# abcouwer-jpl/zsc

Hardware: AMD Instinct MI355X
Metric: deflate level-6 uncompressed MB/s in, Canterbury-like x4096 per GPU (higher is better)
Workload: dtype u8

## Files before the change

### __graft_entry__.py

```python
from __future__ import annotations

import os
import subprocess
import sys

ROOT = os.path.dirname(os.path.abspath(__file__))
if ROOT not in sys.path:
    sys.path.insert(0, ROOT)


def build() -> None:
    subprocess.run(["make", "-s", "-C", os.path.join(ROOT, "zsc_amd", "csrc")], check=True)
    subprocess.run(["make", "-s", "-C", os.path.join(ROOT, "oracle"), "oracle", "ref"], check=True)
    subprocess.run(["make", "-s", "-C", os.path.join(ROOT, "tests", "emu")], check=True)
    subprocess.run(["make", "-s", "-C", os.path.join(ROOT, "tests", "emu_sections")], check=True)
    subprocess.run(["make", "-s", "-C", os.path.join(ROOT, "tests", "emu_chunks")], check=True)
    subprocess.run(["make", "-s", "-C", os.path.join(ROOT, "tests", "emu_resync")], check=True)
    subprocess.run(["make", "-s", "-C", os.path.join(ROOT, "tests", "emu_index")], check=True)
    subprocess.run(["make", "-s", "-C", os.path.join(ROOT, "tests", "emu_size")], check=True)
    subprocess.run(["make", "-s", "-C", os.path.join(ROOT, "tests", "emu_check")], check=True)
    subprocess.run(["make", "-s", "-C", os.path.join(ROOT, "tests", "emu_dindex")], check=True)
    subprocess.run(["make", "-s", "-C", os.path.join(ROOT, "tests", "emu_verify")], check=True)
    subprocess.run(["make", "-s", "-C", os.path.join(ROOT, "tests", "emu_pack")], check=True)
    subprocess.run(["make", "-s", "-C", os.path.join(ROOT, "tests", "emu_pipe")], check=True)
    subprocess.run(["make", "-s", "-C", os.path.join(ROOT, "tests", "emu_sort")], check=True)
    subprocess.run(["make", "-s", "-C", os.path.join(ROOT, "tests", "emu_lazy")], check=True)
    subprocess.run(["make", "-s", "-C", os.path.join(ROOT, "tests", "c_caller")], check=True)
    import zsc_amd


def smoke() -> None:
    import zsc_amd
    from zsc_amd import corpus
    from oracle.oracle_py import Oracle

    print("device:", zsc_amd.device_info())
    oracle = Oracle()
    bufs = [corpus.make_buffer(kind, size, 7 + i) for i, (kind, size) in enumerate(
        [("text", 70000), ("bitmap", 40000), ("table", 20000), ("random", 5000), ("zero", 3000),
         ("token", 257), ("text", 0)])]
    rc, outs, stats = zsc_amd.compress_batch(bufs, level=6)
    assert rc == 0, rc
    for i, (src, got, st) in enumerate(zip(bufs, outs, stats)):
        orc, want, _ = oracle.compress(src, 6)
        assert st == orc == 0, (i, st, orc)
        assert got == want, f"buffer {i}: GPU stream differs from the oracle ({len(got)} vs {len(want)} bytes)"
    rc, one = zsc_amd.compress(bufs[0], level=9)
    assert rc == 0 and one == oracle.compress(bufs[0], 9)[1]
    rc, back, used, istat = zsc_amd.uncompress_batch(outs, [len(b) for b in bufs])
    assert rc == 0 and all(s == 0 for s in istat), (rc, istat)
    assert back == bufs and used == [len(o) for o in outs]
    print("smoke ok:", [len(o) for o in outs])


if __name__ == "__main__":
    build()
    if len(sys.argv) > 1 and sys.argv[1] == "smoke":
        smoke()
```

### zsc_amd/csrc/huff_plan.h

```cpp
#ifndef ZSC_HUFF_PLAN_H
#define ZSC_HUFF_PLAN_H

#include "wave.h"
#include "zsc_dev.h"

#define HP_LCODES 286
#define HP_DCODES 30
#define HP_BLCODES 19
#define HP_HEAP (2 * HP_LCODES + 1)

typedef struct {
    uint32_t freq[HP_HEAP];
    uint16_t parent[HP_HEAP];
    uint16_t len[HP_HEAP];
    uint16_t code[HP_HEAP];
    int max_code;
} HpTree;

typedef struct {
    uint32_t freq[2 * HP_DCODES + 1];
    uint16_t parent[2 * HP_DCODES + 1];
    uint16_t len[2 * HP_DCODES + 2];
    uint16_t code[2 * HP_DCODES + 1];
    int max_code;
} HpTreeD;

typedef struct {
    uint32_t freq[2 * HP_BLCODES + 1];
    uint16_t parent[2 * HP_BLCODES + 1];
    uint16_t len[2 * HP_BLCODES + 1];
    uint16_t code[2 * HP_BLCODES + 1];
    int max_code;
} HpTreeB;

typedef struct {
    HpTree lt;
    HpTreeD dt;
    HpTreeB bt;
    uint16_t heap[HP_HEAP];
    uint8_t depth[HP_HEAP];
    uint16_t per_len[16];
    uint32_t opt_bits, static_bits;
    int heap_n, heap_top;
    uint8_t hdr[ZD_HDR_BYTES];
    uint32_t hdr_acc, hdr_fill, hdr_pos;
} HpLds;

typedef struct {
    uint32_t *freq;
    uint16_t *parent, *len, *code;
    int *max_code;
    int elems, max_len, extra_from, has_static, is_dist;
    int kind;
} HpView;

DEV int hp_extra(int kind, int sym)
{
    if (kind == 0) {
        if (sym < 265 || sym == 285)
            return 0;
        return (sym - 261) >> 2;
    }
    if (kind == 1)
        return sym < 4 ? 0 : (sym >> 1) - 1;
    return sym == 16 ? 2 : sym == 17 ? 3 : sym == 18 ? 7 : 0;
}

DEV uint32_t hp_static_llen(uint32_t c)
{
    return c < 144 ? 8u : c < 256 ? 9u : c < 280 ? 7u : 8u;
}

DEV uint32_t hp_len_code(uint32_t lc)
{
    if (lc < 8)
        return lc;
    if (lc == 255)
        return 28;
    uint32_t e = 29u - (uint32_t)__builtin_clz(lc);
    return 4u * e + 4u + ((lc >> e) & 3u);
}

DEV uint32_t hp_dist_code(uint32_t d)
{
    if (d < 4)
        return d;
    uint32_t e = 30u - (uint32_t)__builtin_clz(d);
    return 2u * e + 2u + ((d >> e) & 1u);
}

DEV uint32_t hp_len_base(uint32_t c)
{
    if (c < 8)
        return c;
    if (c == 28)
        return 0;
    uint32_t e = (c - 4) >> 2;
    return (4u + ((c - 4) & 3u)) << e;
}

DEV uint32_t hp_dist_base(uint32_t c)
{
    if (c < 4)
        return c;
    uint32_t e = (c >> 1) - 1;
    return (2u + (c & 1u)) << e;
}

DEV uint32_t hp_bitrev(uint32_t v, int bits)
{
    uint32_t r = 0;
    while (bits-- > 0) {
        r = (r << 1) | (v & 1u);
        v >>= 1;
    }
    return r;
}

DEV int hp_before(const HpView &t, const uint8_t *depth, int a, int b)
{
    return t.freq[a] < t.freq[b] || (t.freq[a] == t.freq[b] && depth[a] <= depth[b]);
}

DEV void hp_sift(HpLds *h, const HpView &t, int k)
{
    int v = h->heap[k];
    for (int j = k << 1; j <= h->heap_n; j <<= 1) {
        if (j < h->heap_n && hp_before(t, h->depth, h->heap[j + 1], h->heap[j]))
            j++;
        if (hp_before(t, h->depth, v, h->heap[j]))
            break;
        h->heap[k] = h->heap[j];
        k = j;
    }
    h->heap[k] = (uint16_t)v;
}

DEV void hp_build(HpLds *h, const HpView &t)
{
    int top = -1;
    h->heap_n = 0;
    h->heap_top = HP_HEAP;
    for (int n = 0; n < t.elems; n++) {
        if (t.freq[n]) {
            h->heap[++h->heap_n] = (uint16_t)(top = n);
            h->depth[n] = 0;
        } else {
            t.len[n] = 0;
        }
    }
    while (h->heap_n < 2) {
        int node = top < 2 ? ++top : 0;
        h->heap[++h->heap_n] = (uint16_t)node;
        t.freq[node] = 1;
        h->depth[node] = 0;
        h->opt_bits--;
        if (t.has_static)
            h->static_bits -= t.is_dist ? 5u : hp_static_llen((uint32_t)node);
    }
    *t.max_code = top;
    for (int n = h->heap_n / 2; n >= 1; n--)
        hp_sift(h, t, n);

    int node = t.elems;
    do {
        int a = h->heap[1];
        h->heap[1] = h->heap[h->heap_n--];
        hp_sift(h, t, 1);
        int b = h->heap[1];
        h->heap[--h->heap_top] = (uint16_t)a;
        h->heap[--h->heap_top] = (uint16_t)b;
        t.freq[node] = t.freq[a] + t.freq[b];
        h->depth[node] = (uint8_t)((h->depth[a] >= h->depth[b] ? h->depth[a] : h->depth[b]) + 1);
        t.parent[a] = t.parent[b] = (uint16_t)node;
        h->heap[1] = (uint16_t)node++;
        hp_sift(h, t, 1);
    } while (h->heap_n >= 2);
    h->heap[--h->heap_top] = h->heap[1];

    int over = 0;
    for (int b = 0; b < 16; b++)
        h->per_len[b] = 0;
    t.len[h->heap[h->heap_top]] = 0;
    int i;
    for (i = h->heap_top + 1; i < HP_HEAP; i++) {
        int n = h->heap[i];
        int bits = t.len[t.parent[n]] + 1;
        if (bits > t.max_len) {
            bits = t.max_len;
            over++;
        }
        t.len[n] = (uint16_t)bits;
        if (n > top)
            continue;
        h->per_len[bits]++;
        int xb = n >= t.extra_from ? hp_extra(t.kind, n) : 0;
        h->opt_bits += t.freq[n] * (uint32_t)(bits + xb);
        if (t.has_static)
            h->static_bits += t.freq[n] * ((t.is_dist ? 5u : hp_static_llen((uint32_t)n)) + (uint32_t)xb);
    }
    if (over > 0) {
        do {
            int bits = t.max_len - 1;
            while (h->per_len[bits] == 0)
                bits--;
            h->per_len[bits]--;
            h->per_len[bits + 1] += 2;
            h->per_len[t.max_len]--;
            over -= 2;
        } while (over > 0);
        for (int bits = t.max_len; bits != 0; bits--) {
            int n = h->per_len[bits];
            while (n != 0) {
                int m = h->heap[--i];
                if (m > top)
                    continue;
                if (t.len[m] != (uint16_t)bits) {
                    h->opt_bits += ((uint32_t)bits - t.len[m]) * t.freq[m];
                    t.len[m] = (uint16_t)bits;
                }
                n--;
            }
        }
    }
    uint16_t next[16];
    uint32_t code = 0;
    for (int b = 1; b <= 15; b++) {
        code = (code + h->per_len[b - 1]) << 1;
        next[b] = (uint16_t)code;
    }
    for (int n = 0; n <= top; n++) {
        int l = t.len[n];
        if (l)
            t.code[n] = (uint16_t)hp_bitrev(next[l]++, l);
    }
}

DEV void hp_scan(HpLds *h, uint16_t *len, int max_code)
{
    int prev = -1, next = len[0], count = 0, hi = 7, lo = 4;
    if (next == 0) {
        hi = 138;
        lo = 3;
    }
    len[max_code + 1] = 0xffff;
    for (int n = 0; n <= max_code; n++) {
        int cur = next;
        next = len[n + 1];
        if (++count < hi && cur == next)
            continue;
        if (count < lo)
            h->bt.freq[cur] += (uint32_t)count;
        else if (cur != 0) {
            if (cur != prev)
                h->bt.freq[cur]++;
            h->bt.freq[16]++;
        } else if (count <= 10)
            h->bt.freq[17]++;
        else
            h->bt.freq[18]++;
        count = 0;
        prev = cur;
        if (next == 0) {
            hi = 138;
            lo = 3;
        } else if (cur == next) {
            hi = 6;
            lo = 3;
        } else {
            hi = 7;
            lo = 4;
        }
    }
}

DEV void hp_put(HpLds *h, uint32_t value, int nbits)
{
    h->hdr_acc |= value << h->hdr_fill;
    h->hdr_fill += (uint32_t)nbits;
    while (h->hdr_fill >= 8) {
        h->hdr[h->hdr_pos++] = (uint8_t)h->hdr_acc;
        h->hdr_acc >>= 8;
        h->hdr_fill -= 8;
    }
}

DEV void hp_send_lengths(HpLds *h, const uint16_t *len, int max_code)
{
    int prev = -1, next = len[0], count = 0, hi = 7, lo = 4;
    if (next == 0) {
        hi = 138;
        lo = 3;
    }
    for (int n = 0; n <= max_code; n++) {
        int cur = next;
        next = len[n + 1];
        if (++count < hi && cur == next)
            continue;
        if (count < lo) {
            do
                hp_put(h, h->bt.code[cur], h->bt.len[cur]);
            while (--count != 0);
        } else if (cur != 0) {
            if (cur != prev) {
                hp_put(h, h->bt.code[cur], h->bt.len[cur]);
                count--;
            }
            hp_put(h, h->bt.code[16], h->bt.len[16]);
            hp_put(h, (uint32_t)(count - 3), 2);
        } else if (count <= 10) {
            hp_put(h, h->bt.code[17], h->bt.len[17]);
            hp_put(h, (uint32_t)(count - 3), 3);
        } else {
            hp_put(h, h->bt.code[18], h->bt.len[18]);
            hp_put(h, (uint32_t)(count - 11), 7);
        }
        count = 0;
        prev = cur;
        if (next == 0) {
            hi = 138;
            lo = 3;
        } else if (cur == next) {
            hi = 6;
            lo = 3;
        } else {
            hi = 7;
            lo = 4;
        }
    }
}

DEV void huff_plan_block(const uint32_t *syms, const ZdBlockRec *rec, uint32_t strategy,
                         ZdBlockPlan *plan, HpLds *h)
{
    const uint32_t count = rec->sym_count;
    for (int i = 0; i < HP_HEAP; i += WAVE) {
        FOR_LANES
        {
            if (i + LANE < HP_HEAP)
                h->lt.freq[i + LANE] = 0;
        }
    }
    FOR_LANES
    {
        if (LANE < 2 * HP_DCODES + 1)
            h->dt.freq[LANE] = 0;
        if (LANE < 2 * HP_BLCODES + 1)
            h->bt.freq[LANE] = 0;
    }
    for (uint32_t s = 0; s < count; s += WAVE) {
        FOR_LANES
        {
            uint32_t i = s + (uint32_t)LANE;
            if (i < count) {
                uint32_t v = syms[i];
                uint32_t dist = v >> 16, lc = v & 0xff;
                if (dist == 0) {
                    LDS_ADD_U32(&h->lt.freq[lc], 1u);
                } else {
                    LDS_ADD_U32(&h->lt.freq[257 + hp_len_code(lc)], 1u);
                    LDS_ADD_U32(&h->dt.freq[hp_dist_code(dist - 1)], 1u);
                }
            }
        }
    }
    WAVE_SYNC();
    int last_bl = 0;
    uint32_t type = ZD_BT_DYNAMIC;
    ON_LANE0
    {
        h->lt.freq[256] = 1;
        h->opt_bits = h->static_bits = 0;
        HpView vl = {h->lt.freq, h->lt.parent, h->lt.len, h->lt.code, &h->lt.max_code,
                     HP_LCODES, 15, 257, 1, 0, 0};
        HpView vd = {h->dt.freq, h->dt.parent, h->dt.len, h->dt.code, &h->dt.max_code,
                     HP_DCODES, 15, 0, 1, 1, 1};
        HpView vb = {h->bt.freq, h->bt.parent, h->bt.len, h->bt.code, &h->bt.max_code,
                     HP_BLCODES, 7, 0, 0, 0, 2};
        hp_build(h, vl);
        hp_build(h, vd);
        hp_scan(h, h->lt.len, h->lt.max_code);
        hp_scan(h, h->dt.len, h->dt.max_code);
        hp_build(h, vb);
        const uint8_t order[19] = {16, 17, 18, 0, 8, 7, 9, 6, 10, 5, 11, 4, 12, 3, 13, 2, 14, 1, 15};
        for (last_bl = HP_BLCODES - 1; last_bl >= 3; last_bl--)
            if (h->bt.len[order[last_bl]] != 0)
                break;
        h->opt_bits += 3u * ((uint32_t)last_bl + 1u) + 5u + 5u + 4u;

        uint32_t opt_bytes = (h->opt_bits + 3 + 7) >> 3;
        const uint32_t static_bytes = (h->static_bits + 3 + 7) >> 3;
        if (static_bytes <= opt_bytes)
            opt_bytes = static_bytes;
        if (rec->in_len + 4 <= opt_bytes && rec->stored_ok)
            type = ZD_BT_STORED;
        else if (strategy == 4 || static_bytes == opt_bytes)
            type = ZD_BT_STATIC;
        else
            type = ZD_BT_DYNAMIC;

        h->hdr_acc = h->hdr_fill = h->hdr_pos = 0;
        if (type == ZD_BT_DYNAMIC) {
            hp_put(h, (uint32_t)(h->lt.max_code + 1 - 257), 5);
            hp_put(h, (uint32_t)(h->dt.max_code + 1 - 1), 5);
            hp_put(h, (uint32_t)(last_bl + 1 - 4), 4);
            for (int r = 0; r <= last_bl; r++)
                hp_put(h, h->bt.len[order[r]], 3);
            hp_send_lengths(h, h->lt.len, h->lt.max_code);
            hp_send_lengths(h, h->dt.len, h->dt.max_code);
        }
        plan->type = type;
        plan->hdr_bits = h->hdr_pos * 8 + h->hdr_fill;
        if (h->hdr_fill)
            h->hdr[h->hdr_pos] = (uint8_t)h->hdr_acc;
        plan->body_bits = type == ZD_BT_DYNAMIC ? 3u + h->opt_bits
                          : type == ZD_BT_STATIC ? 3u + h->static_bits : 0u;
        plan->bit_off = 0;
    }
    WAVE_SYNC();
    for (int i = 0; i < HP_LCODES; i += WAVE) {
        FOR_LANES
        {
            int s = i + LANE;
            if (s < HP_LCODES) {
                int used = s <= h->lt.max_code && h->lt.len[s] != 0;
                plan->lcode[s] = used ? h->lt.code[s] : (uint16_t)0;
                plan->llen[s] = used ? (uint8_t)h->lt.len[s] : (uint8_t)0;
            }
        }
    }
    FOR_LANES
    {
        if (LANE < HP_DCODES) {
            int used = LANE <= h->dt.max_code && h->dt.len[LANE] != 0;
            plan->dcode[LANE] = used ? h->dt.code[LANE] : (uint16_t)0;
            plan->dlen[LANE] = used ? (uint8_t)h->dt.len[LANE] : (uint8_t)0;
        }
    }
    for (int i = 0; i < (int)ZD_HDR_BYTES; i += WAVE) {
        FOR_LANES
        {
            if (i + LANE < (int)ZD_HDR_BYTES)
                plan->hdr[i + LANE] = h->hdr[i + LANE];
        }
    }
}

#endif
```

Before: 7576.

## Parallelize Huffman plan construction across the wave with packed heap keys

Reworks per-block Huffman tree planning. Heap entries become packed freq/depth/node words, so comparisons are single integer compares and the parent arrays go away. Leaf collection, bit-cost sums and canonical code assignment now run across all lanes using ballot, popcount and wave reductions instead of serial loops on lane 0. The histogram loop issues several symbol loads per lane, and the header bit writer flushes 32-bit words straight into the plan. It also adds an emulator test target. The risk is packed-field overflow (frequency capped near 2^17, checked only by an emulator assert) and subtle tie-break changes that could break bit-exactness with the oracle.

```diff
diff --git a/__graft_entry__.py b/__graft_entry__.py
--- a/__graft_entry__.py
+++ b/__graft_entry__.py
@@ -25,6 +25,7 @@
     subprocess.run(["make", "-s", "-C", os.path.join(ROOT, "tests", "emu_pipe")], check=True)
     subprocess.run(["make", "-s", "-C", os.path.join(ROOT, "tests", "emu_sort")], check=True)
     subprocess.run(["make", "-s", "-C", os.path.join(ROOT, "tests", "emu_lazy")], check=True)
+    subprocess.run(["make", "-s", "-C", os.path.join(ROOT, "tests", "emu_huff")], check=True)
     subprocess.run(["make", "-s", "-C", os.path.join(ROOT, "tests", "c_caller")], check=True)
     import zsc_amd
 
diff --git a/zsc_amd/csrc/huff_plan.h b/zsc_amd/csrc/huff_plan.h
--- a/zsc_amd/csrc/huff_plan.h
+++ b/zsc_amd/csrc/huff_plan.h
@@ -3,56 +3,64 @@
 
 #include "wave.h"
 #include "zsc_dev.h"
+#ifdef ZSC_WAVE_EMU
+#include <assert.h>
+#define HP_ASSERT(x) assert(x)
+#else
+#define HP_ASSERT(x) ((void)0)
+#endif
+
+#ifndef HP_PATH
+#define HP_PATH(id) ((void)0)
+#endif
 
 #define HP_LCODES 286
 #define HP_DCODES 30
 #define HP_BLCODES 19
 #define HP_HEAP (2 * HP_LCODES + 1)
 
+#define HP_NODE_MASK 1023u
+#define HP_WORD(freq, depth, node) (((uint32_t)(freq) << 15) | ((uint32_t)(depth) << 10) | (uint32_t)(node))
+#define HP_KEY(w) ((w) >> 10)
+#define HP_FREQ(w) ((w) >> 15)
+#define HP_DEPTH(w) (((w) >> 10) & 31u)
+#define HP_NO_SYM 0xffffffffu
+#ifndef HP_HIST_LOADS
+#define HP_HIST_LOADS 4
+#endif
+
 typedef struct {
-    uint32_t freq[HP_HEAP];
-    uint16_t parent[HP_HEAP];
-    uint16_t len[HP_HEAP];
-    uint16_t code[HP_HEAP];
-    int max_code;
-} HpTree;
-
-typedef struct {
-    uint32_t freq[2 * HP_DCODES + 1];
-    uint16_t parent[2 * HP_DCODES + 1];
-    uint16_t len[2 * HP_DCODES + 2];
-    uint16_t code[2 * HP_DCODES + 1];
-    int max_code;
-} HpTreeD;
-
-typedef struct {
-    uint32_t freq[2 * HP_BLCODES + 1];
-    uint16_t parent[2 * HP_BLCODES + 1];
-    uint16_t len[2 * HP_BLCODES + 1];
-    uint16_t code[2 * HP_BLCODES + 1];
-    int max_code;
-} HpTreeB;
-
-typedef struct {
-    HpTree lt;
-    HpTreeD dt;
-    HpTreeB bt;
-    uint16_t heap[HP_HEAP];
-    uint8_t depth[HP_HEAP];
-    uint16_t per_len[16];
-    uint32_t opt_bits, static_bits;
-    int heap_n, heap_top;
-    uint8_t hdr[ZD_HDR_BYTES];
-    uint32_t hdr_acc, hdr_fill, hdr_pos;
+    uint32_t heap[HP_HEAP + 1];
+    uint32_t lfreq[HP_LCODES];
+    uint32_t dfreq[HP_DCODES];
+    uint32_t bfreq[HP_BLCODES];
+    uint32_t bsend[HP_BLCODES];
+    uint32_t per_len[16];
+    uint8_t llen[HP_HEAP + 3];
+    uint8_t dlen[2 * HP_DCODES + 4];
+    uint8_t blen[2 * HP_BLCODES + 2];
 } HpLds;
 
-typedef struct {
-    uint32_t *freq;
-    uint16_t *parent, *len, *code;
-    int *max_code;
-    int elems, max_len, extra_from, has_static, is_dist;
-    int kind;
-} HpView;
+template <int KIND> struct HpTree;
+template <> struct HpTree<0> {
+    enum { elems = HP_LCODES, max_len = 15, has_static = 1 };
+};
+template <> struct HpTree<1> {
+    enum { elems = HP_DCODES, max_len = 15, has_static = 1 };
+};
+template <> struct HpTree<2> {
+    enum { elems = HP_BLCODES, max_len = 7, has_static = 0 };
+};
+
+DEV uint32_t *hp_freq(HpLds *h, int kind)
+{
+    return kind == 0 ? h->lfreq : kind == 1 ? h->dfreq : h->bfreq;
+}
+
+DEV uint8_t *hp_len(HpLds *h, int kind)
+{
+    return kind == 0 ? h->llen : kind == 1 ? h->dlen : h->blen;
+}
 
 DEV int hp_extra(int kind, int sym)
 {
@@ -117,148 +125,246 @@
     return r;
 }
 
-DEV int hp_before(const HpView &t, const uint8_t *depth, int a, int b)
-{
-    return t.freq[a] < t.freq[b] || (t.freq[a] == t.freq[b] && depth[a] <= depth[b]);
-}
-
-DEV void hp_sift(HpLds *h, const HpView &t, int k)
-{
-    int v = h->heap[k];
-    for (int j = k << 1; j <= h->heap_n; j <<= 1) {
-        if (j < h->heap_n && hp_before(t, h->depth, h->heap[j + 1], h->heap[j]))
+DEV void hp_sift(uint32_t *heap, int n, int k, uint32_t v)
+{
+    for (int j = k << 1; j <= n; j <<= 1) {
+        uint32_t c = heap[j];
+        const uint32_t c1 = heap[j + 1];
+        if (j < n && HP_KEY(c1) <= HP_KEY(c)) {
+            c = c1;
             j++;
-        if (hp_before(t, h->depth, v, h->heap[j]))
+        }
+        if (HP_KEY(v) <= HP_KEY(c))
             break;
-        h->heap[k] = h->heap[j];
+        heap[k] = c;
         k = j;
     }
-    h->heap[k] = (uint16_t)v;
-}
-
-DEV void hp_build(HpLds *h, const HpView &t)
-{
-    int top = -1;
-    h->heap_n = 0;
-    h->heap_top = HP_HEAP;
-    for (int n = 0; n < t.elems; n++) {
-        if (t.freq[n]) {
-            h->heap[++h->heap_n] = (uint16_t)(top = n);
-            h->depth[n] = 0;
-        } else {
-            t.len[n] = 0;
-        }
-    }
-    while (h->heap_n < 2) {
-        int node = top < 2 ? ++top : 0;
-        h->heap[++h->heap_n] = (uint16_t)node;
-        t.freq[node] = 1;
-        h->depth[node] = 0;
-        h->opt_bits--;
-        if (t.has_static)
-            h->static_bits -= t.is_dist ? 5u : hp_static_llen((uint32_t)node);
-    }
-    *t.max_code = top;
-    for (int n = h->heap_n / 2; n >= 1; n--)
-        hp_sift(h, t, n);
-
-    int node = t.elems;
+    heap[k] = v;
+}
+
+template <int KIND>
+DEV void hp_heap_and_lengths(HpLds *h, int n, int top)
+{
+    typedef HpTree<KIND> T;
+    uint32_t *heap = h->heap;
+    uint8_t *len = hp_len(h, KIND);
+    for (int k = n / 2; k >= 1; k--)
+        hp_sift(heap, n, k, heap[k]);
+
+    int node = T::elems, ht = HP_HEAP;
     do {
-        int a = h->heap[1];
-        h->heap[1] = h->heap[h->heap_n--];
-        hp_sift(h, t, 1);
-        int b = h->heap[1];
-        h->heap[--h->heap_top] = (uint16_t)a;
-        h->heap[--h->heap_top] = (uint16_t)b;
-        t.freq[node] = t.freq[a] + t.freq[b];
-        h->depth[node] = (uint8_t)((h->depth[a] >= h->depth[b] ? h->depth[a] : h->depth[b]) + 1);
-        t.parent[a] = t.parent[b] = (uint16_t)node;
-        h->heap[1] = (uint16_t)node++;
-        hp_sift(h, t, 1);
-    } while (h->heap_n >= 2);
-    h->heap[--h->heap_top] = h->heap[1];
+        const uint32_t a = heap[1];
+        const uint32_t last = heap[n];
+        n--;
+        hp_sift(heap, n, 1, last);
+        const uint32_t b = heap[1];
+        heap[--ht] = ((uint32_t)node << 10) | (a & HP_NODE_MASK);
+        heap[--ht] = ((uint32_t)node << 10) | (b & HP_NODE_MASK);
+        const uint32_t da = HP_DEPTH(a), db = HP_DEPTH(b);
+        const uint32_t depth = (da >= db ? da : db) + 1u, freq = HP_FREQ(a) + HP_FREQ(b);
+        HP_ASSERT(depth < 32u && freq < (1u << 17));
+        hp_sift(heap, n, 1, HP_WORD(freq, depth, node));
+        node++;
+    } while (n >= 2);
+    const int root = (int)(heap[1] & HP_NODE_MASK);
 
     int over = 0;
-    for (int b = 0; b < 16; b++)
-        h->per_len[b] = 0;
-    t.len[h->heap[h->heap_top]] = 0;
-    int i;
-    for (i = h->heap_top + 1; i < HP_HEAP; i++) {
-        int n = h->heap[i];
-        int bits = t.len[t.parent[n]] + 1;
-        if (bits > t.max_len) {
-            bits = t.max_len;
+    len[root] = 0;
+    uint32_t w = heap[ht];
+    for (int i = ht; i < HP_HEAP; i++) {
+        const uint32_t wn = heap[i + 1];
+        int bits = len[w >> 10] + 1;
+        if (bits > (int)T::max_len) {
+            bits = T::max_len;
             over++;
         }
-        t.len[n] = (uint16_t)bits;
-        if (n > top)
-            continue;
-        h->per_len[bits]++;
-        int xb = n >= t.extra_from ? hp_extra(t.kind, n) : 0;
-        h->opt_bits += t.freq[n] * (uint32_t)(bits + xb);
-        if (t.has_static)
-            h->static_bits += t.freq[n] * ((t.is_dist ? 5u : hp_static_llen((uint32_t)n)) + (uint32_t)xb);
+        len[w & HP_NODE_MASK] = (uint8_t)bits;
+        w = wn;
     }
     if (over > 0) {
+        HP_PATH(1 + KIND);
+        uint32_t *per_len = h->per_len;
+        for (int b = 0; b < 16; b++)
+            per_len[b] = 0;
+        for (int i = ht; i < HP_HEAP; i++) {
+            const int m = (int)(heap[i] & HP_NODE_MASK);
+            if (m <= top)
+                per_len[len[m]]++;
+        }
         do {
-            int bits = t.max_len - 1;
-            while (h->per_len[bits] == 0)
+            int bits = T::max_len - 1;
+            while (per_len[bits] == 0)
                 bits--;
-            h->per_len[bits]--;
-            h->per_len[bits + 1] += 2;
-            h->per_len[t.max_len]--;
+            per_len[bits]--;
+            per_len[bits + 1] += 2;
+            per_len[T::max_len]--;
             over -= 2;
         } while (over > 0);
-        for (int bits = t.max_len; bits != 0; bits--) {
-            int n = h->per_len[bits];
-            while (n != 0) {
-                int m = h->heap[--i];
+        int i = HP_HEAP;
+        for (int bits = T::max_len; bits != 0; bits--) {
+            uint32_t k = per_len[bits];
+            while (k != 0) {
+                const int m = (int)(heap[--i] & HP_NODE_MASK);
                 if (m > top)
                     continue;
-                if (t.len[m] != (uint16_t)bits) {
-                    h->opt_bits += ((uint32_t)bits - t.len[m]) * t.freq[m];
-                    t.len[m] = (uint16_t)bits;
+                len[m] = (uint8_t)bits;
+                k--;
+            }
+        }
+    }
+}
+
+template <int KIND>
+DEV int hp_build(HpLds *h, ZdBlockPlan *plan, uint32_t &opt_bits, uint32_t &static_bits)
+{
+    typedef HpTree<KIND> T;
+    enum { NCH = (T::elems + WAVE - 1) / WAVE };
+    uint32_t *const freq = hp_freq(h, KIND);
+    uint8_t *const len = hp_len(h, KIND);
+    int top = -1, n = 0;
+    for (int c = 0; c < NCH; c++) {
+        LANEVAR(uint32_t, f);
+        FOR_LANES
+        {
+            const int s = c * WAVE + LANE;
+            LV(f) = s < (int)T::elems ? freq[s] : 0u;
+            if (s < (int)T::elems)
+                len[s] = 0;
+        }
+        const uint64_t m = BALLOT(f);
+        FOR_LANES
+        {
+            if (LV(f))
+                h->heap[n + 1 + POPC64(m & ((1ull << LANE) - 1ull))] = HP_WORD(LV(f), 0, c * WAVE + LANE);
+        }
+        if (m) {
+            n += POPC64(m);
+            top = c * WAVE + 63 - CLZ64(m);
+        }
+    }
+    while (n < 2) {
+        HP_PATH(0);
+        const int node = top < 2 ? ++top : 0;
+        n++;
+        ON_LANE0
+        {
+            h->heap[n] = HP_WORD(1, 0, node);
+            freq[node] = 1;
+        }
+        opt_bits--;
+        if (T::has_static)
+            static_bits -= KIND == 1 ? 5u : hp_static_llen((uint32_t)node);
+    }
+    WAVE_SYNC();
+    ON_LANE0
+    {
+        hp_heap_and_lengths<KIND>(h, n, top);
+    }
+    WAVE_SYNC();
+
+    LANEARR(uint32_t, ln, NCH);
+    LANEARR(uint32_t, cd, NCH);
+    LANEVAR(uint64_t, bits);
+    FOR_LANES
+    {
+        LV(bits) = 0;
+    }
+    UNROLL_FULL
+    for (int c = 0; c < NCH; c++) {
+        FOR_LANES
+        {
+            const int s = c * WAVE + LANE;
+            uint32_t l = 0;
+            if (s < (int)T::elems) {
+                l = len[s];
+                const uint32_t fr = freq[s], xb = (uint32_t)hp_extra(KIND, s);
+                LV(bits) += (uint64_t)(fr * (l + xb));
+                if (T::has_static)
+                    LV(bits) += (uint64_t)(fr * ((KIND == 1 ? 5u : hp_static_llen((uint32_t)s)) + xb)) << 32;
+            }
+            LVA(ln, c) = l;
+            LVA(cd, c) = 0;
+        }
+    }
+    const uint64_t total = WAVE_SUM(bits);
+    opt_bits += (uint32_t)total;
+    static_bits += (uint32_t)(total >> 32);
+
+    uint32_t code = 0, count = 0;
+    for (int l = 1; l <= (int)T::max_len; l++) {
+        code = (code + count) << 1;
+        uint32_t run = code;
+        UNROLL_FULL
+        for (int c = 0; c < NCH; c++) {
+            LANEVAR(uint32_t, is);
+            FOR_LANES
+            {
+                LV(is) = LVA(ln, c) == (uint32_t)l;
+            }
+            const uint64_t m = BALLOT(is);
+            FOR_LANES
+            {
+                if (LV(is))
+                    LVA(cd, c) = run + (uint32_t)POPC64(m & ((1ull << LANE) - 1ull));
+            }
+            run += (uint32_t)POPC64(m);
+        }
+        count = run - code;
+    }
+    UNROLL_FULL
+    for (int c = 0; c < NCH; c++) {
+        FOR_LANES
+        {
+            const int s = c * WAVE + LANE;
+            if (s < (int)T::elems) {
+                const uint32_t l = LVA(ln, c);
+                const uint32_t rev = l ? BREV32(LVA(cd, c)) >> (32u - l) : 0u;
+                if (KIND == 0) {
+                    plan->lcode[s] = (uint16_t)rev;
+                    plan->llen[s] = (uint8_t)l;
+                } else if (KIND == 1) {
+                    plan->dcode[s] = (uint16_t)rev;
+                    plan->dlen[s] = (uint8_t)l;
+                } else {
+                    h->bsend[s] = rev | (l << 16);
                 }
-                n--;
-            }
-        }
-    }
-    uint16_t next[16];
-    uint32_t code = 0;
-    for (int b = 1; b <= 15; b++) {
-        code = (code + h->per_len[b - 1]) << 1;
-        next[b] = (uint16_t)code;
-    }
-    for (int n = 0; n <= top; n++) {
-        int l = t.len[n];
-        if (l)
-            t.code[n] = (uint16_t)hp_bitrev(next[l]++, l);
-    }
-}
-
-DEV void hp_scan(HpLds *h, uint16_t *len, int max_code)
-{
-    int prev = -1, next = len[0], count = 0, hi = 7, lo = 4;
+            }
+        }
+    }
+    return top;
+}
+
+DEV uint32_t hp_len_at(const uint8_t *len, uint32_t &word, int i)
+{
+    if ((i & 3) == 0)
+        __builtin_memcpy(&word, __builtin_assume_aligned(len + i, 4), 4);
+    return (word >> ((i & 3) * 8)) & 0xffu;
+}
+
+DEV void hp_scan(HpLds *h, uint8_t *len, int max_code)
+{
+    len[max_code + 1] = 0xff;
+    uint32_t word = 0;
+    int prev = -1, next = (int)hp_len_at(len, word, 0), count = 0, hi = 7, lo = 4;
     if (next == 0) {
         hi = 138;
         lo = 3;
     }
-    len[max_code + 1] = 0xffff;
     for (int n = 0; n <= max_code; n++) {
         int cur = next;
-        next = len[n + 1];
+        next = (int)hp_len_at(len, word, n + 1);
         if (++count < hi && cur == next)
             continue;
         if (count < lo)
-            h->bt.freq[cur] += (uint32_t)count;
+            LDS_ADD_U32(&h->bfreq[cur], (uint32_t)count);
         else if (cur != 0) {
             if (cur != prev)
-                h->bt.freq[cur]++;
-            h->bt.freq[16]++;
+                LDS_ADD_U32(&h->bfreq[cur], 1u);
+            LDS_ADD_U32(&h->bfreq[16], 1u);
         } else if (count <= 10)
-            h->bt.freq[17]++;
+            LDS_ADD_U32(&h->bfreq[17], 1u);
         else
-            h->bt.freq[18]++;
+            LDS_ADD_U32(&h->bfreq[18], 1u);
         count = 0;
         prev = cur;
         if (next == 0) {
@@ -274,46 +380,57 @@
     }
 }
 
-DEV void hp_put(HpLds *h, uint32_t value, int nbits)
-{
-    h->hdr_acc |= value << h->hdr_fill;
-    h->hdr_fill += (uint32_t)nbits;
-    while (h->hdr_fill >= 8) {
-        h->hdr[h->hdr_pos++] = (uint8_t)h->hdr_acc;
-        h->hdr_acc >>= 8;
-        h->hdr_fill -= 8;
-    }
-}
-
-DEV void hp_send_lengths(HpLds *h, const uint16_t *len, int max_code)
-{
-    int prev = -1, next = len[0], count = 0, hi = 7, lo = 4;
+typedef struct {
+    uint64_t acc;
+    uint32_t fill, pos;
+    uint8_t *out;
+} HpBits;
+
+DEV void hp_put(HpBits &w, uint32_t value, int nbits)
+{
+    w.acc |= (uint64_t)value << w.fill;
+    w.fill += (uint32_t)nbits;
+    if (w.fill >= 32) {
+        const uint32_t lo = (uint32_t)w.acc;
+        __builtin_memcpy(__builtin_assume_aligned(w.out + w.pos, 4), &lo, 4);
+        w.pos += 4;
+        w.acc >>= 32;
+        w.fill -= 32;
+    }
+}
+
+DEV void hp_send_lengths(HpLds *h, HpBits &w, const uint8_t *len, int max_code)
+{
+    uint32_t word = 0;
+    int prev = -1, next = (int)hp_len_at(len, word, 0), count = 0, hi = 7, lo = 4;
     if (next == 0) {
         hi = 138;
         lo = 3;
     }
     for (int n = 0; n <= max_code; n++) {
         int cur = next;
-        next = len[n + 1];
+        next = (int)hp_len_at(len, word, n + 1);
         if (++count < hi && cur == next)
             continue;
         if (count < lo) {
+            const uint32_t s = h->bsend[cur];
             do
-                hp_put(h, h->bt.code[cur], h->bt.len[cur]);
+                hp_put(w, s & 0xffffu, (int)(s >> 16));
             while (--count != 0);
         } else if (cur != 0) {
             if (cur != prev) {
-                hp_put(h, h->bt.code[cur], h->bt.len[cur]);
+                const uint32_t s = h->bsend[cur];
+                hp_put(w, s & 0xffffu, (int)(s >> 16));
                 count--;
             }
-            hp_put(h, h->bt.code[16], h->bt.len[16]);
-            hp_put(h, (uint32_t)(count - 3), 2);
+            const uint32_t s = h->bsend[16];
+            hp_put(w, (s & 0xffffu) | ((uint32_t)(count - 3) << (s >> 16)), (int)(s >> 16) + 2);
         } else if (count <= 10) {
-            hp_put(h, h->bt.code[17], h->bt.len[17]);
-            hp_put(h, (uint32_t)(count - 3), 3);
+            const uint32_t s = h->bsend[17];
+            hp_put(w, (s & 0xffffu) | ((uint32_t)(count - 3) << (s >> 16)), (int)(s >> 16) + 3);
         } else {
-            hp_put(h, h->bt.code[18], h->bt.len[18]);
-            hp_put(h, (uint32_t)(count - 11), 7);
+            const uint32_t s = h->bsend[18];
+            hp_put(w, (s & 0xffffu) | ((uint32_t)(count - 11) << (s >> 16)), (int)(s >> 16) + 7);
         }
         count = 0;
         prev = cur;
@@ -330,120 +447,126 @@
     }
 }
 
+DEV uint32_t hp_bl_order(int r)
+{
+    const uint64_t a = 16ull | 17ull << 5 | 18ull << 10 | 0ull << 15 | 8ull << 20 | 7ull << 25 | 9ull << 30 |
+                       6ull << 35 | 10ull << 40 | 5ull << 45 | 11ull << 50 | 4ull << 55;
+    const uint64_t b = 12ull | 3ull << 5 | 13ull << 10 | 2ull << 15 | 14ull << 20 | 1ull << 25 | 15ull << 30;
+    return (uint32_t)((r < 12 ? a >> (5 * r) : b >> (5 * (r - 12))) & 31u);
+}
+
 DEV void huff_plan_block(const uint32_t *syms, const ZdBlockRec *rec, uint32_t strategy,
                          ZdBlockPlan *plan, HpLds *h)
 {
     const uint32_t count = rec->sym_count;
-    for (int i = 0; i < HP_HEAP; i += WAVE) {
-        FOR_LANES
-        {
-            if (i + LANE < HP_HEAP)
-                h->lt.freq[i + LANE] = 0;
-        }
-    }
-    FOR_LANES
-    {
-        if (LANE < 2 * HP_DCODES + 1)
-            h->dt.freq[LANE] = 0;
-        if (LANE < 2 * HP_BLCODES + 1)
-            h->bt.freq[LANE] = 0;
-    }
-    for (uint32_t s = 0; s < count; s += WAVE) {
-        FOR_LANES
-        {
-            uint32_t i = s + (uint32_t)LANE;
-            if (i < count) {
-                uint32_t v = syms[i];
-                uint32_t dist = v >> 16, lc = v & 0xff;
-                if (dist == 0) {
-                    LDS_ADD_U32(&h->lt.freq[lc], 1u);
+    for (int i = 0; i < HP_LCODES; i += WAVE) {
+        FOR_LANES
+        {
+            if (i + LANE < HP_LCODES)
+                h->lfreq[i + LANE] = i + LANE == 256 ? 1u : 0u;
+        }
+    }
+    for (int i = 0; i < HP_DCODES; i += WAVE) {
+        FOR_LANES
+        {
+            if (i + LANE < HP_DCODES)
+                h->dfreq[i + LANE] = 0;
+            if (i + LANE < HP_BLCODES)
+                h->bfreq[i + LANE] = 0;
+        }
+    }
+    WAVE_SYNC();
+    for (uint32_t s = 0; s < count; s += HP_HIST_LOADS * WAVE) {
+        FOR_LANES
+        {
+            uint32_t v[HP_HIST_LOADS];
+            UNROLL_FULL
+            for (int k = 0; k < HP_HIST_LOADS; k++) {
+                const uint32_t i = s + (uint32_t)(k * WAVE + LANE);
+                v[k] = i < count ? syms[i] : HP_NO_SYM;
+            }
+            UNROLL_FULL
+            for (int k = 0; k < HP_HIST_LOADS; k++) {
+                const uint32_t dist = v[k] >> 16, lc = v[k] & 0xff;
+                if (v[k] == HP_NO_SYM) {
+                } else if (dist == 0) {
+                    LDS_ADD_U32(&h->lfreq[lc], 1u);
                 } else {
-                    LDS_ADD_U32(&h->lt.freq[257 + hp_len_code(lc)], 1u);
-                    LDS_ADD_U32(&h->dt.freq[hp_dist_code(dist - 1)], 1u);
+                    LDS_ADD_U32(&h->lfreq[257 + hp_len_code(lc)], 1u);
+                    LDS_ADD_U32(&h->dfreq[hp_dist_code(dist - 1)], 1u);
                 }
             }
         }
     }
     WAVE_SYNC();
-    int last_bl = 0;
-    uint32_t type = ZD_BT_DYNAMIC;
+    uint32_t opt_bits = 0, static_bits = 0;
+    const int lmax = hp_build<0>(h, plan, opt_bits, static_bits);
+    const int dmax = hp_build<1>(h, plan, opt_bits, static_bits);
     ON_LANE0
     {
-        h->lt.freq[256] = 1;
-        h->opt_bits = h->static_bits = 0;
-        HpView vl = {h->lt.freq, h->lt.parent, h->lt.len, h->lt.code, &h->lt.max_code,
-                     HP_LCODES, 15, 257, 1, 0, 0};
-        HpView vd = {h->dt.freq, h->dt.parent, h->dt.len, h->dt.code, &h->dt.max_code,
-                     HP_DCODES, 15, 0, 1, 1, 1};
-        HpView vb = {h->bt.freq, h->bt.parent, h->bt.len, h->bt.code, &h->bt.max_code,
-                     HP_BLCODES, 7, 0, 0, 0, 2};
-        hp_build(h, vl);
-        hp_build(h, vd);
-        hp_scan(h, h->lt.len, h->lt.max_code);
-        hp_scan(h, h->dt.len, h->dt.max_code);
-        hp_build(h, vb);
-        const uint8_t order[19] = {16, 17, 18, 0, 8, 7, 9, 6, 10, 5, 11, 4, 12, 3, 13, 2, 14, 1, 15};
-        for (last_bl = HP_BLCODES - 1; last_bl >= 3; last_bl--)
-            if (h->bt.len[order[last_bl]] != 0)
-                break;
-        h->opt_bits += 3u * ((uint32_t)last_bl + 1u) + 5u + 5u + 4u;
-
-        uint32_t opt_bytes = (h->opt_bits + 3 + 7) >> 3;
-        const uint32_t static_bytes = (h->static_bits + 3 + 7) >> 3;
-        if (static_bytes <= opt_bytes)
-            opt_bytes = static_bytes;
-        if (rec->in_len + 4 <= opt_bytes && rec->stored_ok)
-            type = ZD_BT_STORED;
-        else if (strategy == 4 || static_bytes == opt_bytes)
-            type = ZD_BT_STATIC;
-        else
-            type = ZD_BT_DYNAMIC;
-
-        h->hdr_acc = h->hdr_fill = h->hdr_pos = 0;
+        hp_scan(h, h->llen, lmax);
+        hp_scan(h, h->dlen, dmax);
+    }
+    WAVE_SYNC();
+    hp_build<2>(h, plan, opt_bits, static_bits);
+    WAVE_SYNC();
+    int last_bl = 0;
+    uint64_t bl_bits = 0;
+    for (int i = 0; i < HP_BLCODES; i += WAVE) {
+        LANEVAR(uint32_t, bl);
+        FOR_LANES
+        {
+            LV(bl) = i + LANE < HP_BLCODES ? h->bsend[hp_bl_order(i + LANE)] >> 16 : 0u;
+        }
+        const uint64_t m = BALLOT(bl);
+        if (m)
+            last_bl = i + 63 - CLZ64(m);
+        LANEVAR(uint64_t, part);
+        FOR_LANES
+        {
+            LV(part) = i + LANE < HP_BLCODES ? (uint64_t)LV(bl) << (3 * (i + LANE)) : 0ull;
+        }
+        bl_bits += WAVE_SUM(part);
+    }
+    if (last_bl < 3)
+        last_bl = 3;
+    opt_bits += 3u * ((uint32_t)last_bl + 1u) + 5u + 5u + 4u;
+
+    uint32_t opt_bytes = (opt_bits + 3 + 7) >> 3;
+    const uint32_t static_bytes = (static_bits + 3 + 7) >> 3;
+    if (static_bytes <= opt_bytes)
+        opt_bytes = static_bytes;
+    uint32_t type;
+    if (rec->in_len + 4 <= opt_bytes && rec->stored_ok)
+        type = ZD_BT_STORED;
+    else if (strategy == 4 || static_bytes == opt_bytes)
+        type = ZD_BT_STATIC;
+    else
+        type = ZD_BT_DYNAMIC;
+    ON_LANE0
+    {
+        HP_PATH(4 + type);
+        HpBits w = {0, 0, 0, plan->hdr};
         if (type == ZD_BT_DYNAMIC) {
-            hp_put(h, (uint32_t)(h->lt.max_code + 1 - 257), 5);
-            hp_put(h, (uint32_t)(h->dt.max_code + 1 - 1), 5);
-            hp_put(h, (uint32_t)(last_bl + 1 - 4), 4);
-            for (int r = 0; r <= last_bl; r++)
-                hp_put(h, h->bt.len[order[r]], 3);
-            hp_send_lengths(h, h->lt.len, h->lt.max_code);
-            hp_send_lengths(h, h->dt.len, h->dt.max_code);
+            hp_put(w, (uint32_t)(lmax + 1 - 257) | (uint32_t)(dmax + 1 - 1) << 5 | (uint32_t)(last_bl + 1 - 4) << 10, 14);
+            const int nb = 3 * (last_bl + 1);
+            const uint64_t sent = nb < 64 ? bl_bits & ((1ull << nb) - 1ull) : bl_bits;
+            hp_put(w, (uint32_t)sent, nb < 32 ? nb : 32);
+            if (nb > 32)
+                hp_put(w, (uint32_t)(sent >> 32), nb - 32);
+            hp_send_lengths(h, w, h->llen, lmax);
+            hp_send_lengths(h, w, h->dlen, dmax);
         }
         plan->type = type;
-        plan->hdr_bits = h->hdr_pos * 8 + h->hdr_fill;
-        if (h->hdr_fill)
-            h->hdr[h->hdr_pos] = (uint8_t)h->hdr_acc;
-        plan->body_bits = type == ZD_BT_DYNAMIC ? 3u + h->opt_bits
-                          : type == ZD_BT_STATIC ? 3u + h->static_bits : 0u;
+        plan->hdr_bits = w.pos * 8 + w.fill;
+        if (w.fill) {
+            const uint32_t lo = (uint32_t)w.acc;
+            __builtin_memcpy(__builtin_assume_aligned(w.out + w.pos, 4), &lo, 4);
+        }
+        plan->body_bits = type == ZD_BT_DYNAMIC ? 3u + opt_bits : type == ZD_BT_STATIC ? 3u + static_bits : 0u;
         plan->bit_off = 0;
     }
     WAVE_SYNC();
-    for (int i = 0; i < HP_LCODES; i += WAVE) {
-        FOR_LANES
-        {
-            int s = i + LANE;
-            if (s < HP_LCODES) {
-                int used = s <= h->lt.max_code && h->lt.len[s] != 0;
-                plan->lcode[s] = used ? h->lt.code[s] : (uint16_t)0;
-                plan->llen[s] = used ? (uint8_t)h->lt.len[s] : (uint8_t)0;
-            }
-        }
-    }
-    FOR_LANES
-    {
-        if (LANE < HP_DCODES) {
-            int used = LANE <= h->dt.max_code && h->dt.len[LANE] != 0;
-            plan->dcode[LANE] = used ? h->dt.code[LANE] : (uint16_t)0;
-            plan->dlen[LANE] = used ? (uint8_t)h->dt.len[LANE] : (uint8_t)0;
-        }
-    }
-    for (int i = 0; i < (int)ZD_HDR_BYTES; i += WAVE) {
-        FOR_LANES
-        {
-            if (i + LANE < (int)ZD_HDR_BYTES)
-                plan->hdr[i + LANE] = h->hdr[i + LANE];
-        }
-    }
 }
 
 #endif
```

New measurement: 7688, median of 6. +1.5%, better.
